# lim0606/pytorch-ardae-vae

Measured on AMD Instinct MI355X. Metric: AR-DAE-VAE train-steps/sec (batch 512, nz_cdae 256) on dbMNIST, higher is better.
Workload: dtype f32; 1 GPU; BASELINE config #2: MNISTIPVAE mlp z=32 h=256 + cDAE mlp-grad h=256 L=3, global batch 512, nz_cdae 256 (131072 rows), dynamic binarisation on device, 1 cDAE + 1 VAE update per step; global_batch=512, nz_cdae=256, per_gpu_batch=512, parallelism=dp1

## Files before the change

pytorch-ardae-vae_amd/csrc/linear_wide.hip:

```cpp
#include <string.h>

#include "linear_wide_kernel.h"

namespace ardae {
namespace wide {

int wide_grid(int ntiles, int ncp) {
  static const char* genv = debug_knob("ARDAE_WIDE_GRID");
  int g = genv ? atoi(genv) : 256;
  g -= g % ncp;
  return ntiles < g ? ntiles : g;
}

}

namespace {

using namespace wide;

bool al16w(const void* p) { return (reinterpret_cast<uintptr_t>(p) & 15) == 0; }

int wide_panels(const LinArgs& a, int& nch, int& nj) {
  if (a.nsrc != 1) return 0;
  if (a.src[0].K == 256) { nch = 8; nj = 2; return 4; }
  if (a.src[0].K == 32) { nch = 4; nj = 2; return 1; }
  if (a.src[0].K == 512) { nch = 8; nj = 1; return 8; }
  if (a.src[0].K == 1024) { nch = 8; nj = 1; return 16; }
  return 0;
}

template <int EPI, int ACT, bool F1, bool F2>
int launch_wide_nch(const LinArgs& a, hipStream_t st) {
  int nch = 0, nj = 0;
  const int np = wide_panels(a, nch, nj);
  if (np == 16) {
    if constexpr (ACT == ACT_SOFTPLUS && !F1 && (EPI == EPI_ACT || (EPI == EPI_DACT && !F2))) return launch_wide<8, 16, 1, EPI, ACT, F1, F2>(a, st);
    ARDAE_CHECK_ARG(false, "linear_wide: K = 1024 is instantiated for softplus ACT / DACT-without-Q epilogues only");
  }
  if (np == 8) return launch_wide<8, 8, 1, EPI, ACT, F1, F2>(a, st);
  if (nch == 4) return launch_wide<4, 1, 2, EPI, ACT, F1, F2>(a, st);
  return launch_wide<8, 4, 2, EPI, ACT, F1, F2>(a, st);
}

template <int EPI, int ACT>
int launch_wide_flags(const LinArgs& a, hipStream_t st) {
  if constexpr (EPI == EPI_ACT) {
    const bool y2 = a.Y2 != nullptr, rs = a.rowscale != nullptr;
    if (y2 && rs) return launch_wide_nch<EPI, ACT, true, true>(a, st);
    if (y2) return launch_wide_nch<EPI, ACT, true, false>(a, st);
    if (rs) return launch_wide_nch<EPI, ACT, false, true>(a, st);
    return launch_wide_nch<EPI, ACT, false, false>(a, st);
  } else if constexpr (EPI == EPI_DACT) {
    if (a.Q) return launch_wide_nch<EPI, ACT, true, false>(a, st);
    return launch_wide_nch<EPI, ACT, false, false>(a, st);
  } else {
    return launch_wide_nch<EPI, ACT, false, false>(a, st);
  }
}

}

bool linear_wide_eligible(const LinArgs& a, int epi) {
  int nch = 0, nj = 0;
  if (wide_panels(a, nch, nj) == 0) return false;
  const int wgcols = 128 * nj;
  if (a.M <= 0 || (a.M % WBM) || a.Nout <= 0 || (a.Nout % wgcols)) return false;
  if ((int64_t)(a.M / WBM) * (a.Nout / wgcols) < 128) return false;
  for (int s = 0; s < a.nsrc; ++s) {
    if (a.src[s].K % 32 || (a.src[s].ld & 3) || !al16w(a.src[s].x)) return false;
    if ((int64_t)a.src[s].ld * a.M * 4 >= (int64_t)1 << 32) return false;
  }
  if (epi == EPI_DAE_LOSS) return false;
  if (a.colsum && linear_row_tile(a.M, a.Nout) != WBM) return false;
  if (a.src[0].K == 1024) {
    if (a.act != ACT_SOFTPLUS) return false;
    if (!((epi == EPI_ACT && !a.Y2) || (epi == EPI_DACT && !a.Q))) return false;
  }
  if (a.act != ACT_NONE && a.act != ACT_RELU && a.act != ACT_SOFTPLUS) return false;
  if (epi == EPI_CHAIN && a.act != ACT_SOFTPLUS) return false;
  if (256 % (a.Nout / wgcols)) return false;
  if (epi == EPI_ACT && a.rowbias) {
    if (a.rows_per_group <= 0) return false;
    if (a.rows_per_group % WBM && (a.rows_per_group < WBM || a.M % a.rows_per_group || a.colsum)) return false;
  }
  if (epi == EPI_ACT && a.rowscale && !a.rowscale_w) return false;
  const int64_t ldmax = std::max<int64_t>({a.ldY, a.ldY2, a.ldS, a.ldR, a.ldQ});
  if (ldmax * a.M * 4 >= (int64_t)1 << 32) return false;
  return true;
}

bool linear_wide_layers_eligible(const LinArgs* L, int nl, int epi) {
  static const bool on = !(debug_knob("ARDAE_WIDE_LAYERS") && atoi(debug_knob("ARDAE_WIDE_LAYERS")) == 0);
  if (!on || nl < 2 || nl > WIDE_MAXL || !(epi == EPI_ACT || epi == EPI_DACT || epi == EPI_CHAIN)) return false;
  const LinArgs& f = L[0];
  if (f.act != ACT_SOFTPLUS && !(f.act == ACT_RELU && epi != EPI_CHAIN)) return false;
  for (int l = 0; l < nl; ++l) {
    const LinArgs& a = L[l];
    if (!linear_wide_eligible(a, epi)) return false;
    if (a.M != f.M || a.Nout != 256 || a.nsrc != 1 || a.src[0].K != 256 || a.act != f.act || !a.Y) return false;
    if (l > 0 && (a.src[0].x != L[l - 1].Y || a.src[0].ld != L[l - 1].ldY)) return false;
    if (epi == EPI_ACT && (a.rowbias || a.rowscale || a.Y2)) return false;
    if (epi == EPI_DACT && ((a.Q != nullptr) != (f.Q != nullptr))) return false;
    if (epi == EPI_CHAIN && (!a.Y2 || !a.R)) return false;
  }
  return true;
}

int launch_linear_wide_layers(const LinArgs* L, int nl, int epi, hipStream_t st) {
  ARDAE_CHECK_ARG(linear_wide_layers_eligible(L, nl, epi), "linear_wide_layers: run not eligible");
  const int act = L[0].act;
  if (epi == EPI_ACT) return act == ACT_SOFTPLUS ? launch_wide_layers<8, 4, 2, EPI_ACT, ACT_SOFTPLUS, false, false>(L, nl, st)
                                                 : launch_wide_layers<8, 4, 2, EPI_ACT, ACT_RELU, false, false>(L, nl, st);
  if (epi == EPI_CHAIN) return launch_wide_layers<8, 4, 2, EPI_CHAIN, ACT_SOFTPLUS, false, false>(L, nl, st);
  if (L[0].Q) return act == ACT_SOFTPLUS ? launch_wide_layers<8, 4, 2, EPI_DACT, ACT_SOFTPLUS, true, false>(L, nl, st)
                                         : launch_wide_layers<8, 4, 2, EPI_DACT, ACT_RELU, true, false>(L, nl, st);
  return act == ACT_SOFTPLUS ? launch_wide_layers<8, 4, 2, EPI_DACT, ACT_SOFTPLUS, false, false>(L, nl, st)
                             : launch_wide_layers<8, 4, 2, EPI_DACT, ACT_RELU, false, false>(L, nl, st);
}

int launch_linear_wide(const LinArgs& a, int epi, hipStream_t st) {
  switch (epi) {
    case EPI_ACT:
      if (a.act == ACT_NONE) return launch_wide_flags<EPI_ACT, ACT_NONE>(a, st);
      if (a.act == ACT_RELU) return launch_wide_flags<EPI_ACT, ACT_RELU>(a, st);
      if (a.act == ACT_SOFTPLUS) return launch_wide_flags<EPI_ACT, ACT_SOFTPLUS>(a, st);
      break;
    case EPI_DACT:
      if (a.act == ACT_NONE) return launch_wide_flags<EPI_DACT, ACT_NONE>(a, st);
      if (a.act == ACT_RELU) return launch_wide_flags<EPI_DACT, ACT_RELU>(a, st);
      if (a.act == ACT_SOFTPLUS) return launch_wide_flags<EPI_DACT, ACT_SOFTPLUS>(a, st);
      break;
    case EPI_CHAIN:
      if (a.act == ACT_SOFTPLUS) return launch_wide_flags<EPI_CHAIN, ACT_SOFTPLUS>(a, st);
      break;
  }
  ARDAE_CHECK_ARG(false, "linear_wide: unsupported epilogue/activation combination (epi=%d act=%d)", epi, a.act);
  return -1;
}

}
```

pytorch-ardae-vae_amd/csrc/linear_wide_kernel.h:

```cpp
#pragma once
#include <stdlib.h>

#include <algorithm>
#include <type_traits>

#include "linear.h"
#include "profile.h"

#define ARDAE_NT_LD " nt"
#define ARDAE_NT_ST " nt"
namespace ardae {
namespace wide {

constexpr int WBM = 64;
constexpr int WLDW = 68;
constexpr int WBUF_BYTES = WBM * WLDW * 4;
constexpr int NBUF = 3;

typedef __attribute__((address_space(3))) float lds_f32;

template <int OFF>
__device__ __forceinline__ void gload4(f32x4& dst, unsigned voff, const float* sbase) {
  asm volatile("s_nop 4\n\tglobal_load_dwordx4 %0, %1, %2 offset:%3" : "=v"(dst) : "v"(voff), "s"(sbase), "n"(OFF) : "memory");
}
template <int OFF, bool NOP = true>
__device__ __forceinline__ void gload1(float& dst, unsigned voff, const float* sbase) {
  if (NOP) asm volatile("s_nop 4\n\tglobal_load_dword %0, %1, %2 offset:%3" : "=v"(dst) : "v"(voff), "s"(sbase), "n"(OFF) : "memory");
  else asm volatile("global_load_dword %0, %1, %2 offset:%3" : "=v"(dst) : "v"(voff), "s"(sbase), "n"(OFF) : "memory");
}
template <bool NOP = true>
__device__ __forceinline__ void gstore1(unsigned voff, float v, float* sbase) {
  if (NOP) asm volatile("s_nop 4\n\tglobal_store_dword %0, %1, %2" ::"v"(voff), "v"(v), "s"(sbase) : "memory");
  else asm volatile("global_store_dword %0, %1, %2" ::"v"(voff), "v"(v), "s"(sbase) : "memory");
}
typedef int i32x4 __attribute__((ext_vector_type(4)));
__device__ __forceinline__ i32x4 make_rsrc(const void* p, unsigned bytes) {
  const unsigned long long a = (unsigned long long)p;
  i32x4 r;
  r[0] = (int)(unsigned)a;
  r[1] = (int)((unsigned)(a >> 32) & 0xffffu);
  r[2] = (int)bytes;
  r[3] = 0x00020000;
  return r;
}
template <int OFF, int H>
__device__ __forceinline__ void bload1(f32x2& dst, unsigned voff, const i32x4& rsrc, unsigned soff) {
  asm volatile("s_nop 4\n\tbuffer_load_dword %0, %1, %2, %3 offen offset:%4" ARDAE_NT_LD : "+v"(dst[H]) : "v"(voff), "s"(rsrc), "s"(soff), "n"(OFF) : "memory");
}
__device__ __forceinline__ void bstore1(unsigned voff, float v, const i32x4& rsrc, unsigned soff) {
  asm volatile("s_nop 4\n\tbuffer_store_dword %0, %1, %2, %3 offen" ARDAE_NT_ST ::"v"(v), "v"(voff), "s"(rsrc), "s"(soff) : "memory");
}
template <int OFF>
__device__ __forceinline__ void lds_read4(f32x4& dst, unsigned addr) {
  asm volatile("ds_read_b128 %0, %1 offset:%2" : "=v"(dst) : "v"(addr), "n"(OFF) : "memory");
}
template <int OFF>
__device__ __forceinline__ void lds_write4(unsigned addr, const f32x4& v) {
  asm volatile("ds_write_b128 %0, %1 offset:%2" ::"v"(addr), "v"(v), "n"(OFF) : "memory");
}
template <int VM, int NX>
__device__ __forceinline__ void wait_panel(f32x4 (&x)[NX]) {
  if (NX == 4) asm volatile("s_waitcnt vmcnt(%4)" : "+v"(x[0]), "+v"(x[1]), "+v"(x[2]), "+v"(x[3]) : "n"(VM) : "memory");
  else asm volatile("s_waitcnt vmcnt(%2)" : "+v"(x[0]), "+v"(x[1]) : "n"(VM) : "memory");
}
template <int VM>
__device__ __forceinline__ void wait16(f32x2* v) {
  asm volatile("s_waitcnt vmcnt(%8)" : "+v"(v[0]), "+v"(v[1]), "+v"(v[2]), "+v"(v[3]), "+v"(v[4]), "+v"(v[5]), "+v"(v[6]), "+v"(v[7]) : "n"(VM) : "memory");
}

template <int NCH>
struct PanelGeo {
  static constexpr int C4 = 2 * NCH;
  static constexpr int RPP = 256 / C4;
  static constexpr int NX = WBM / RPP;
};


template <int NCH, int NX>
__device__ __forceinline__ void store_panel(const f32x4 (&xv)[NX], unsigned waddr) {
  using PG = PanelGeo<NCH>;
  lds_write4<0>(waddr, xv[0]);
  lds_write4<PG::RPP * WLDW * 4>(waddr, xv[1]);
  if (NX == 4) {
    lds_write4<2 * PG::RPP * WLDW * 4>(waddr, xv[2]);
    lds_write4<3 * PG::RPP * WLDW * 4>(waddr, xv[3]);
  }
}
template <int OFF>
__device__ __forceinline__ void bload4(f32x4& dst, unsigned voff, const i32x4& rsrc, unsigned soff) {
  asm volatile("s_nop 4\n\tbuffer_load_dwordx4 %0, %1, %2, %3 offen offset:%4" : "=v"(dst) : "v"(voff), "s"(rsrc), "s"(soff), "n"(OFF) : "memory");
}
__device__ __forceinline__ void gload4_agpr(f32x4& dst, unsigned voff, const float* sbase) {
  asm volatile("s_nop 4\n\tglobal_load_dwordx4 %0, %1, %2" : "=a"(dst) : "v"(voff), "s"(sbase) : "memory");
}
template <int VM, int NJ>
__device__ __forceinline__ void wait_slab(f32x4 (&b)[NJ]) {
  if constexpr (NJ == 2) asm volatile("s_waitcnt vmcnt(%2)" : "+a"(b[0]), "+a"(b[1]) : "n"(VM) : "memory");
  else asm volatile("s_waitcnt vmcnt(%1)" : "+a"(b[0]) : "n"(VM) : "memory");
}
template <bool FIRST, bool LAST>
__device__ __forceinline__ void mfma_vab(f32x16& acc, float a, float b) {
  if (FIRST) asm volatile("v_mfma_f32_32x32x2_f32 %0, %1, %2, 0" : "=v"(acc) : "v"(a), "a"(b));
  else if (LAST) asm volatile("v_mfma_f32_32x32x2_f32 %0, %1, %2, %0\n\ts_nop 15\n\ts_nop 3" : "+v"(acc) : "v"(a), "a"(b));
  else asm volatile("v_mfma_f32_32x32x2_f32 %0, %1, %2, %0" : "+v"(acc) : "v"(a), "a"(b));
}

constexpr int wide_slots(int NCH, int NP, int NJ) { return (NJ * NCH * NP * 4 <= 256) ? NCH * NP : 64 / NJ; }

template <int NCH, int NP, int NJ, int NLT, int NST, bool HP>
struct Sched {
  static constexpr int NX = PanelGeo<NCH>::NX;
  static constexpr int G = NP * NCH;
  static constexpr int SLOTS = wide_slots(NCH, NP, NJ);
  static constexpr bool ROLL = SLOTS < G;
  static constexpr bool DEFER = NP >= 2;
  static constexpr int NSTO = (DEFER && HP) ? 32 * NJ * NST : 0;
  static constexpr int NLD = 32 * NJ * NLT;
  static constexpr int XW = NCH - 3, BAR = NCH - 2;
  static constexpr int GE = G >= 16 ? G - 5 : G - 1;
  static constexpr int GS = (NSTO + NLD) == 0 ? 0 : NLD == 0 ? GE : (GE * NSTO + (NSTO + NLD) / 2) / (NSTO + NLD);
  static constexpr int GRB = NLD == 0 ? GE - 1 : GS;
  static constexpr int DS = GS > 0 ? GS : 1, DL = GE > GS ? GE - GS : 1;
  static constexpr int st_lo(int g) { return g >= GS ? NSTO : NSTO * g / DS; }
  static constexpr int st_hi(int g) { return g >= GS ? NSTO : NSTO * (g + 1) / DS; }
  static constexpr int ld_lo(int g) { return g < GS ? 0 : g >= GE ? NLD : NLD * (g - GS) / DL; }
  static constexpr int ld_hi(int g) { return g < GS ? 0 : g >= GE ? NLD : NLD * (g - GS + 1) / DL; }
  static constexpr int n_rb(int g) { return g == GRB ? NJ : 0; }
  static constexpr int n_sl(int g) { return ROLL ? NJ : 0; }
  static constexpr int vmem(int g) { return (st_hi(g) - st_lo(g)) + n_rb(g) + (ld_hi(g) - ld_lo(g)) + n_sl(g); }
  static constexpr int vm_panel(int p) {
    int n = 0;
    for (int k = 0; k < XW; ++k) n += vmem(p * NCH + k);
    return n > 63 ? 63 : n;
  }
  static constexpr int vm_slab(int p, int c) {
    const int g = p * NCH + c;
    int n = ((ROLL ? SLOTS : G) - 1 - g) * NJ + NX * (c > 0 ? p + 1 : p);
    if (n < 0) n = 0;
    for (int k = 0; k < g; ++k) n += vmem(k);
    return n > 63 ? 63 : n;
  }
};

template <int EPI, int ACT, bool F1, bool F2, int NJ_ = 2>
struct WideEpi {
  static constexpr int NJ = NJ_;
  static constexpr int NLT = EPI == EPI_ACT ? (F2 ? 1 : 0) : EPI == EPI_DACT ? (F1 ? 2 : 1) : 2;
  static constexpr int NST = EPI == EPI_ACT ? (F1 ? 2 : 1) : EPI == EPI_DACT ? 1 : 2;
  static constexpr bool SIGMA_OPERAND = EPI == EPI_ACT;
  static constexpr bool CHAIN = EPI == EPI_CHAIN;

  const LinArgs& a;
  unsigned vY, vY2, vL0, vL1, vRS, vC;
  i32x4 rY, rY2, rL0, rL1, rRS;
  unsigned sY, sY2, sL0, sL1;
  float bcol0, wsig0, wfc0; unsigned pad_; float bcol1, wsig1, wfc1;
  int colw_loaded;

  __device__ __forceinline__ WideEpi(const LinArgs& a_, int lane) : a(a_), colw_loaded(-1) {
    const int l31 = lane & 31, hh = lane >> 5;
    vY = (unsigned)((4 * hh * a.ldY + l31) * 4);
    vY2 = NST == 2 ? (unsigned)((4 * hh * (a.Y2 ? a.ldY2 : a.ldY) + l31) * 4) : 0u;
    vL0 = (EPI != EPI_ACT) ? (unsigned)((4 * hh * a.ldS + l31) * 4) : 0u;
    vL1 = (EPI == EPI_CHAIN) ? (unsigned)((4 * hh * a.ldR + l31) * 4) : (EPI == EPI_DACT && F1) ? (unsigned)((4 * hh * a.ldQ + l31) * 4) : 0u;
    vRS = (unsigned)(16 * hh);
    vC = (unsigned)(l31 * 4);
    bcol0 = bcol1 = wsig0 = wsig1 = wfc0 = wfc1 = 0.f;
    const unsigned M = (unsigned)a.M;
    const float* y2 = a.Y2 ? a.Y2 : a.Y;
    const int ld2 = a.Y2 ? a.ldY2 : a.ldY;
    sY = (unsigned)a.ldY * 4u; sY2 = (unsigned)ld2 * 4u;
    rY = make_rsrc(a.Y, M * sY);
    rY2 = make_rsrc(y2, M * sY2);
    const float* t0 = EPI != EPI_ACT ? a.S : a.Y;
    const float* t1 = EPI == EPI_CHAIN ? a.R : (EPI == EPI_DACT && F1) ? a.Q : a.Y;
    sL0 = (unsigned)(EPI != EPI_ACT ? a.ldS : a.ldY) * 4u;
    sL1 = (unsigned)(EPI == EPI_CHAIN ? a.ldR : (EPI == EPI_DACT && F1) ? a.ldQ : a.ldY) * 4u;
    rL0 = make_rsrc(t0, M * sL0);
    rL1 = make_rsrc(t1, M * sL1);
    rRS = make_rsrc((EPI == EPI_ACT && a.rowscale) ? a.rowscale : a.src[0].x, M * 4u);
  }

  __device__ __forceinline__ void column_operands(int colw, int lane) {
    if (EPI != EPI_ACT || colw == colw_loaded) return;
    colw_loaded = colw;
    const int l31 = lane & 31;
#pragma unroll
    for (int j = 0; j < NJ; ++j) {
      const int col = colw + 32 * j + l31;
      const float b = a.bias ? a.bias[col] : 0.f;
      const float w = (F2 && a.rowscale_w) ? a.rowscale_w[col] : 0.f;
      const float f = (F1 && a.R) ? a.R[col] : 0.f;
      if (j == 0) { bcol0 = b; wsig0 = w; wfc0 = f; } else { bcol1 = b; wsig1 = w; wfc1 = f; }
    }
  }

  template <int JJ>
  __device__ __forceinline__ void issue_rowbias_one(float& rbj, int row0, int colw) const {
    const float* p = (EPI == EPI_ACT && a.rowbias) ? a.rowbias + (size_t)(row0 / a.rows_per_group) * a.rowbias_ld + colw
                                                     : a.Y + (size_t)row0 * a.ldY + colw;
    gload1<128 * JJ>(rbj, vC, p);
  }

  template <int HB>
  __device__ __forceinline__ void math(const f32x16& acc16, f32x2* l0, f32x2* l1, float brow, f32x2& csum) const {
    constexpr int J = HB >> 2, H = HB & 1;
    const float ws = J == 0 ? wsig0 : wsig1, nw = -(J == 0 ? wfc0 : wfc1);
    const f32x2 brow2 = {brow, brow}, wsig2 = {ws, ws}, nwfc2 = {nw, nw};
#pragma unroll
    for (int k = 0; k < 4; ++k) {
      f32x2 v;
      v[0] = acc16[8 * H + 2 * k];
      v[1] = acc16[8 * H + 2 * k + 1];
      f32x2 em;
      if (EPI == EPI_ACT) {
        f32x2 x = v + brow2;
        if (F2 && a.rowscale) x = l0[k] * wsig2 + x;
        const f32x2 y = act_fwd2<ACT>(x);
        if (NST == 2) l1[k] = (F1 && a.Y2) ? nwfc2 * act_d1_2<ACT>(y, em) : y;
        l0[k] = y;
      } else if (EPI == EPI_DACT) {
        const f32x2 d1 = act_d1_2<ACT>(l0[k], em);
        if (F1) asm volatile("v_pk_fma_f32 %0, %1, %2, %3" : "+v"(l0[k]) : "v"(v), "v"(d1), "v"(l1[k]));
        else asm volatile("v_pk_mul_f32 %0, %1, %2" : "+v"(l0[k]) : "v"(v), "v"(d1));
      } else {
        const f32x2 d1 = act_d1_2<ACT>(l0[k], em);
        const f32x2 vem = v * em;
        asm volatile("v_pk_mul_f32 %0, %1, %2" : "+v"(l0[k]) : "v"(v), "v"(d1));
        asm volatile("v_pk_mul_f32 %0, %1, %0" : "+v"(l1[k]) : "v"(vem));
      }
      csum += l0[k];
    }
  }

  template <int HB>
  __device__ __forceinline__ void stores(const f32x2* y, const f32x2* y2, int row0, int colw) const {
    constexpr int J = HB >> 2, I = (HB >> 1) & 1, H = HB & 1;
    const unsigned r0 = (unsigned)(row0 + 32 * I + 16 * H), c4 = (unsigned)(colw + 32 * J) * 4u;
    unsigned oy = r0 * sY + c4;
#pragma unroll
    for (int e = 0; e < 8; ++e) {
      bstore1(vY, y[e >> 1][e & 1], rY, oy);
      oy += (e == 3) ? 5u * sY : sY;
    }
    if (NST == 2) {
      unsigned o2 = r0 * sY2 + c4;
#pragma unroll
      for (int e = 0; e < 8; ++e) {
        bstore1(vY2, y2[e >> 1][e & 1], rY2, o2);
        o2 += (e == 3) ? 5u * sY2 : sY2;
      }
    }
  }

  __device__ __forceinline__ void store_all(const f32x2* y, const f32x2* y2, int row0, int colw) const {
    stores<0>(y + 0, y2 + 0, row0, colw); stores<1>(y + 4, y2 + 4, row0, colw); stores<2>(y + 8, y2 + 8, row0, colw);
    stores<3>(y + 12, y2 + 12, row0, colw);
    if constexpr (NJ == 2) {
      stores<4>(y + 16, y2 + 16, row0, colw); stores<5>(y + 20, y2 + 20, row0, colw);
      stores<6>(y + 24, y2 + 24, row0, colw); stores<7>(y + 28, y2 + 28, row0, colw);
    }
  }

  template <int VM, bool STORE_NOW>
  __device__ __forceinline__ void run(f32x16 (&acc)[2][NJ], f32x2* l0, f32x2* l1, float (&rb)[NJ], int lane, int row0, int colw, int tile_row) const {
    asm volatile("s_waitcnt vmcnt(%2)" : "+v"(rb[0]), "+v"(rb[NJ - 1]) : "n"(VM) : "memory");
    if (NLT >= 1) { wait16<VM>(l0); wait16<VM>(l0 + 8); if (NJ == 2) { wait16<VM>(l0 + 16); wait16<VM>(l0 + 24); } }
    if (NLT == 2) { wait16<VM>(l1); wait16<VM>(l1 + 8); if (NJ == 2) { wait16<VM>(l1 + 16); wait16<VM>(l1 + 24); } }
    const bool has_rb = EPI == EPI_ACT && a.rowbias != nullptr;
    const float br0 = bcol0 + (has_rb ? rb[0] : 0.f), br1 = bcol1 + (has_rb ? rb[NJ - 1] : 0.f);
    f32x2 csum[2] = {f32x2{0.f, 0.f}, f32x2{0.f, 0.f}};
    math<0>(acc[0][0], l0 + 0, l1 + 0, br0, csum[0]); __builtin_amdgcn_sched_barrier(0);
    math<1>(acc[0][0], l0 + 4, l1 + 4, br0, csum[0]); __builtin_amdgcn_sched_barrier(0);
    math<2>(acc[1][0], l0 + 8, l1 + 8, br0, csum[0]); __builtin_amdgcn_sched_barrier(0);
    math<3>(acc[1][0], l0 + 12, l1 + 12, br0, csum[0]); __builtin_amdgcn_sched_barrier(0);
    if constexpr (NJ == 2) {
      math<4>(acc[0][1], l0 + 16, l1 + 16, br1, csum[1]); __builtin_amdgcn_sched_barrier(0);
      math<5>(acc[0][1], l0 + 20, l1 + 20, br1, csum[1]); __builtin_amdgcn_sched_barrier(0);
      math<6>(acc[1][1], l0 + 24, l1 + 24, br1, csum[1]); __builtin_amdgcn_sched_barrier(0);
      math<7>(acc[1][1], l0 + 28, l1 + 28, br1, csum[1]); __builtin_amdgcn_sched_barrier(0);
    }
    if (STORE_NOW) store_all(l0, l1, row0, colw);
    if (a.colsum != nullptr) {
#pragma unroll
      for (int j = 0; j < NJ; ++j) {
        const float c1 = csum[j][0] + csum[j][1];
        const float c2 = c1 + __shfl_xor(c1, 32);
        if (lane < 32) a.colsum[(size_t)tile_row * a.Nout + colw + 32 * j + lane] = c2;
      }
    }
  }
};

template <int NCH, class EPI_T>
struct PanelCtx {
  const EPI_T& epi;
  const i32x4& rX;
  unsigned xvoff, xstep, xsoff_next;
  unsigned raddr, raddr_next, waddr_next;
  int row0, colw, prev_row0;
  const float* wslab;
  unsigned bvoff;
  int kch;
};

template <int C, int P, int NCH, int NP, bool HP, bool FT, class EPI_T>
struct ChunkOps {
  using SC = Sched<NCH, NP, EPI_T::NJ, EPI_T::NLT, EPI_T::NST, HP>;
  static constexpr int NX = PanelGeo<NCH>::NX;
  static constexpr int NLT = EPI_T::NLT, NST = EPI_T::NST, NJ = EPI_T::NJ, NMF = 8 * EPI_T::NJ;
  static constexpr int GC = P * NCH + C;
  static constexpr int n_a = 2, n_x = C == 0 ? NX : 0, n_w = C == SC::XW ? NX : 0, n_st = SC::st_hi(GC) - SC::st_lo(GC), n_rb = SC::n_rb(GC),
                       n_op = SC::ld_hi(GC) - SC::ld_lo(GC), n_sl = SC::n_sl(GC);
  static constexpr int o_a = 0, o_x = o_a + n_a, o_w = o_x + n_x, o_st = o_w + n_w, o_rb = o_st + n_st, o_op = o_rb + n_rb, o_sl = o_op + n_op,
                       total = o_sl + n_sl;
  static constexpr int SLOTS = SC::SLOTS;
  static constexpr int PER = (total + NMF - 1) / NMF;

  struct Ptrs {
    unsigned py, py2, p0, p1;
  };

  template <int K>
  static __device__ __forceinline__ void op(f32x4 (&A)[2][2], f32x4 (&Bw)[SC::SLOTS][EPI_T::NJ], f32x4 (&xv)[NX], f32x2* l0, f32x2* l1, float (&rb)[EPI_T::NJ],
                                            const PanelCtx<NCH, EPI_T>& x, Ptrs& q) {
    using PG = PanelGeo<NCH>;
    const EPI_T& ep = x.epi;
    if constexpr (K >= o_sl) {
      constexpr int j = K - o_sl, GP = (GC + SC::G - 1) % SC::G, GN = (GP + SLOTS) % SC::G;
      asm volatile("s_nop 4\n\tglobal_load_dwordx4 %0, %1, %2" : "+a"(Bw[GP % SLOTS][j]) : "v"(x.bvoff), "s"(x.wslab + ((size_t)j * x.kch + GN) * 256) : "memory");
    } else if constexpr (K < o_x) {
      constexpr int i = K - o_a;
      if constexpr (C + 1 < NCH) lds_read4<(C + 1) * 32 + i * 32 * WLDW * 4>(A[(C + 1) & 1][i], x.raddr);
      else lds_read4<i * 32 * WLDW * 4>(A[0][i], x.raddr_next);
    } else if constexpr (K < o_w) {
      constexpr int u = K - o_x;
      bload4<0>(xv[u], x.xvoff, x.rX, x.xsoff_next + (unsigned)u * x.xstep);
    } else if constexpr (K < o_st) {
      constexpr int u = K - o_w;
      if constexpr (u == 0) wait_panel<SC::vm_panel(P), NX>(xv);
      lds_write4<u * PG::RPP * WLDW * 4>(x.waddr_next, xv[u]);
    } else if constexpr (K < o_rb) {
      constexpr int idx = SC::st_lo(GC) + (K - o_st);
      constexpr int HB = idx / (8 * NST), tns = (idx / 8) % NST, e = idx % 8;
      constexpr int J = HB >> 2, I = (HB >> 1) & 1, H = HB & 1;
      constexpr bool fresh = e == 0 || K == o_st;
      constexpr int roff = 32 * I + 16 * H + (e & 3) + 8 * (e >> 2);
      if constexpr (tns == 0) {
        if constexpr (fresh) q.py = (unsigned)(x.prev_row0 + roff) * ep.sY + (unsigned)(x.colw + 32 * J) * 4u;
        bstore1(ep.vY, l0[4 * HB + (e >> 1)][e & 1], ep.rY, q.py);
        q.py += (e == 3) ? 5u * ep.sY : ep.sY;
      } else {
        if constexpr (fresh) q.py2 = (unsigned)(x.prev_row0 + roff) * ep.sY2 + (unsigned)(x.colw + 32 * J) * 4u;
        bstore1(ep.vY2, l1[4 * HB + (e >> 1)][e & 1], ep.rY2, q.py2);
        q.py2 += (e == 3) ? 5u * ep.sY2 : ep.sY2;
      }
    } else if constexpr (K < o_op) {
      constexpr int k = K - o_rb;
      if constexpr (k == 0) ep.template issue_rowbias_one<0>(rb[0], x.row0, x.colw);
      else ep.template issue_rowbias_one<1>(rb[NJ - 1], x.row0, x.colw);
    } else if constexpr (K < o_sl) {
      constexpr int idx = SC::ld_lo(GC) + (K - o_op);
      constexpr int HB = idx / (8 * NLT), tns = (idx / 8) % NLT, e = idx % 8;
      constexpr int J = HB >> 2, I = (HB >> 1) & 1, H = HB & 1;
      constexpr bool fresh = e == 0 || K == o_op;
      constexpr int roff = 32 * I + 16 * H + (e & 3) + 8 * (e >> 2);
      if constexpr (EPI_T::SIGMA_OPERAND) {
        constexpr int off = ((e & 3) + 8 * (e >> 2)) * 4;
        bload1<off, (e & 1)>(l0[4 * HB + (e >> 1)], ep.vRS, ep.rRS, (unsigned)(x.row0 + 32 * I + 16 * H) * 4u);
      } else if constexpr (tns == 0) {
        if constexpr (fresh) q.p0 = (unsigned)(x.row0 + roff) * ep.sL0 + (unsigned)(x.colw + 32 * J) * 4u;
        bload1<0, (e & 1)>(l0[4 * HB + (e >> 1)], ep.vL0, ep.rL0, q.p0);
        q.p0 += (e == 3) ? 5u * ep.sL0 : ep.sL0;
      } else {
        if constexpr (fresh) q.p1 = (unsigned)(x.row0 + roff) * ep.sL1 + (unsigned)(x.colw + 32 * J) * 4u;
        bload1<0, (e & 1)>(l1[4 * HB + (e >> 1)], ep.vL1, ep.rL1, q.p1);
        q.p1 += (e == 3) ? 5u * ep.sL1 : ep.sL1;
      }
    }
  }

  template <int S, int R = 0>
  static __device__ __forceinline__ void slot(f32x4 (&A)[2][2], f32x4 (&Bw)[SC::SLOTS][EPI_T::NJ], f32x4 (&xv)[NX], f32x2* l0, f32x2* l1, float (&rb)[EPI_T::NJ],
                                              const PanelCtx<NCH, EPI_T>& x, Ptrs& q) {
    if constexpr (R < PER && S * PER + R < total) {
      op<S * PER + R>(A, Bw, xv, l0, l1, rb, x, q);
      slot<S, R + 1>(A, Bw, xv, l0, l1, rb, x, q);
    }
  }

  template <int S>
  static __device__ __forceinline__ void steps(f32x16 (&acc)[2][EPI_T::NJ], f32x4 (&A)[2][2], f32x4 (&Bw)[wide_slots(NCH, NP, EPI_T::NJ)][EPI_T::NJ], f32x4 (&xv)[NX], f32x2* l0, f32x2* l1,
                                               float (&rb)[EPI_T::NJ], const PanelCtx<NCH, EPI_T>& x, Ptrs& q) {
    if constexpr (S < NMF) {
      constexpr int kq = S / (2 * NJ), i = (S / NJ) & 1, j = S % NJ;
      mfma_vab<GC == 0 && kq == 0, GC == NP * NCH - 1 && S == NMF - 1>(acc[i][j], A[C & 1][i][kq], Bw[GC % SLOTS][j][kq]);
      slot<S>(A, Bw, xv, l0, l1, rb, x, q);
      steps<S + 1>(acc, A, Bw, xv, l0, l1, rb, x, q);
    }
  }

  static __device__ __forceinline__ void run(f32x16 (&acc)[2][EPI_T::NJ], f32x4 (&A)[2][2], f32x4 (&Bw)[wide_slots(NCH, NP, EPI_T::NJ)][EPI_T::NJ], f32x4 (&xv)[NX], f32x2* l0, f32x2* l1,
                                             float (&rb)[EPI_T::NJ], const PanelCtx<NCH, EPI_T>& x) {
    asm volatile("s_waitcnt lgkmcnt(0)" : "+v"(A[C & 1][0]), "+v"(A[C & 1][1]) : : "memory");
    if constexpr (FT && GC < SLOTS) wait_slab<SC::vm_slab(P, C), NJ>(Bw[GC % SLOTS]);
    else if constexpr (SC::ROLL) wait_slab<63, NJ>(Bw[GC % SLOTS]);
    if (C == SC::BAR) __builtin_amdgcn_s_barrier();
    Ptrs q{0u, 0u, 0u, 0u};
    steps<0>(acc, A, Bw, xv, l0, l1, rb, x, q);
  }
};

template <int P, int NCH, int NP, bool HP, bool FT, class EPI_T>
__device__ __forceinline__ void panel(f32x16 (&acc)[2][EPI_T::NJ], f32x4 (&A)[2][2], f32x4 (&Bw)[wide_slots(NCH, NP, EPI_T::NJ)][EPI_T::NJ], f32x4 (&xv)[PanelGeo<NCH>::NX], f32x2* l0, f32x2* l1,
                                      float (&rb)[EPI_T::NJ], const PanelCtx<NCH, EPI_T>& x) {
  ChunkOps<0, P, NCH, NP, HP, FT, EPI_T>::run(acc, A, Bw, xv, l0, l1, rb, x);
  ChunkOps<1, P, NCH, NP, HP, FT, EPI_T>::run(acc, A, Bw, xv, l0, l1, rb, x);
  ChunkOps<2, P, NCH, NP, HP, FT, EPI_T>::run(acc, A, Bw, xv, l0, l1, rb, x);
  ChunkOps<3, P, NCH, NP, HP, FT, EPI_T>::run(acc, A, Bw, xv, l0, l1, rb, x);
  if constexpr (NCH == 8) {
    ChunkOps<4, P, NCH, NP, HP, FT, EPI_T>::run(acc, A, Bw, xv, l0, l1, rb, x);
    ChunkOps<5, P, NCH, NP, HP, FT, EPI_T>::run(acc, A, Bw, xv, l0, l1, rb, x);
    ChunkOps<6, P, NCH, NP, HP, FT, EPI_T>::run(acc, A, Bw, xv, l0, l1, rb, x);
    ChunkOps<7, P, NCH, NP, HP, FT, EPI_T>::run(acc, A, Bw, xv, l0, l1, rb, x);
  }
}

template <int P, int NCH, int NP, bool HP, bool FT, class EPI_T, class PX>
__device__ __forceinline__ void tile_panels(f32x16 (&acc)[2][EPI_T::NJ], f32x4 (&A)[2][2], f32x4 (&Bw)[wide_slots(NCH, NP, EPI_T::NJ)][EPI_T::NJ], f32x4 (&xv)[PanelGeo<NCH>::NX], f32x2* l0,
                                            f32x2* l1, float (&rb)[EPI_T::NJ], const EPI_T& epi, const i32x4& rX, unsigned xvoff, unsigned xstep, int& buf,
                                            unsigned rlane, unsigned wlane, int row0, int colw, int prev_row0, int tile, int tnext, const PX& panel_x,
                                            const float* wslab, unsigned bvoff, int kch) {
  if constexpr (P < NP) {
    constexpr bool lastp = P + 1 == NP;
    const int bnext = buf + 1 == NBUF ? 0 : buf + 1;
    const PanelCtx<NCH, EPI_T> x{epi, rX, xvoff, xstep, panel_x(lastp ? tnext : tile, lastp ? 0 : P + 1), rlane + buf * WBUF_BYTES, rlane + bnext * WBUF_BYTES,
                                 wlane + bnext * WBUF_BYTES, row0, colw, prev_row0, wslab, bvoff, kch};
    panel<P, NCH, NP, HP, FT>(acc, A, Bw, xv, l0, l1, rb, x);
    buf = bnext;
    tile_panels<P + 1, NCH, NP, HP, FT>(acc, A, Bw, xv, l0, l1, rb, epi, rX, xvoff, xstep, buf, rlane, wlane, row0, colw, prev_row0, tile, tnext, panel_x, wslab,
                                        bvoff, kch);
  }
}

template <int NCH, int NP, int NJ, int EPI, int ACT, bool F1, bool F2>
__device__ __forceinline__ void wide_body(const LinArgs& a, int nrt, int ncp, int tpg) {
  using PG = PanelGeo<NCH>;
  using EPI_T = WideEpi<EPI, ACT, F1, F2, NJ>;
  using SC = Sched<NCH, NP, NJ, EPI_T::NLT, EPI_T::NST, true>;
  constexpr int NX = PG::NX, G = NP * NCH;
  static_assert(NCH % 2 == 0 && NCH >= 4, "fragment double buffer / XW, BAR chunks");
  constexpr int SLOTS = wide_slots(NCH, NP, NJ);
  static_assert(NJ * SLOTS * 4 <= 256 && G % SLOTS == 0, "the slab window must fit the AGPR file");
  __shared__ float lds[NBUF * WBM * WLDW];

#ifdef ARDAE_STAMPS
  const unsigned long long r_kernel = __builtin_amdgcn_s_memrealtime();
#endif
  const int tid = threadIdx.x, lane = tid & 63;
  const int wave = __builtin_amdgcn_readfirstlane(tid >> 6);
  const int l31 = lane & 31, hh = lane >> 5;

  const unsigned lds0 = (unsigned)(uintptr_t)(lds_f32*)lds;
  const unsigned rlane = lds0 + (unsigned)((l31 * WLDW + hh * 4) * 4);
  const unsigned wlane = lds0 + (unsigned)(((tid / PG::C4) * WLDW + (tid % PG::C4) * 4) * 4);

  const int b = (int)blockIdx.x, nwg = (int)gridDim.x;
  const bool xcd_map = ncp > 1 && nwg % (8 * ncp) == 0;
  const int cp = xcd_map ? (b >> 3) % ncp : b % ncp;
  const int rt0 = xcd_map ? ((b >> 3) / ncp) * 8 + (b & 7) : b / ncp;
  const int rts = nwg / ncp;
  const int colw = (cp * 4 * NJ + wave * NJ) * 32;
  EPI_T epi(a, lane);
  epi.column_operands(colw, lane);

  const unsigned ldx4 = (unsigned)a.src[0].ld * 4u;
  const i32x4 rX = make_rsrc(a.src[0].x, (unsigned)a.M * ldx4);
  const unsigned xvoff = (unsigned)(tid / PG::C4) * ldx4 + (unsigned)(tid % PG::C4) * 16u;
  const unsigned xstep = (unsigned)PG::RPP * ldx4;
  auto tile_row0 = [&](int rt) -> int {
    if (tpg == 0) return rt * WBM;
    const int g = rt / tpg, j = rt - g * tpg;
    const int r = j * WBM, last = a.rows_per_group - WBM;
    return __builtin_amdgcn_readfirstlane(g * a.rows_per_group + (r < last ? r : last));
  };
  auto panel_x = [&](int rt, int p) -> unsigned { return (unsigned)tile_row0(rt) * ldx4 + (unsigned)(p * 8 * NCH) * 4u; };

  f32x4 A[2][2], Bw[SLOTS][NJ], xv[NX];
  f32x2 l0[16 * NJ], l1[16 * NJ];
  float rb[NJ];
#pragma unroll
  for (int i = 0; i < 16 * NJ; ++i) l0[i] = l1[i] = f32x2{0.f, 0.f};
  int tile = rt0;
  const unsigned bvoff = (unsigned)lane * 16u;
  const int kch = a.src[0].K >> 3;
  const float* wslab = a.src[0].wp + (size_t)(cp * 4 * NJ + wave * NJ) * kch * 256;
  {
    const float* wp = wslab;
    const unsigned x0 = panel_x(tile, 0);
#pragma unroll
    for (int u = 0; u < NX; ++u) bload4<0>(xv[u], xvoff, rX, x0 + (unsigned)u * xstep);
#pragma unroll
    for (int g = 0; g < SLOTS; ++g) {
      gload4_agpr(Bw[g][0], bvoff, wp + (size_t)g * 256);
      if constexpr (NJ == 2) gload4_agpr(Bw[g][1], bvoff, wp + ((size_t)kch + g) * 256);
    }
    wait_panel<(NJ * SLOTS > 63 ? 63 : NJ * SLOTS), NX>(xv);
    store_panel<NCH, NX>(xv, wlane);
    asm volatile("s_waitcnt lgkmcnt(0)" ::: "memory");
    __builtin_amdgcn_s_barrier();
    lds_read4<0>(A[0][0], rlane);
    lds_read4<32 * WLDW * 4>(A[0][1], rlane);
  }
  int buf = 0;
  int prev_row0 = -1;
#ifdef ARDAE_STAMPS
  unsigned long long t_k = 0, t_e = 0;
  const unsigned long long t_begin = __builtin_amdgcn_s_memtime();
  const unsigned long long r_begin = __builtin_amdgcn_s_memrealtime();
#endif
  auto do_tile = [&](auto ft_tag) {
    constexpr bool FT = decltype(ft_tag)::value, HP = SC::DEFER && !FT;
#ifdef ARDAE_STAMPS
    const unsigned long long T0 = __builtin_amdgcn_s_memtime();
#endif
    const int tr = tile;
    const int row0 = tile_row0(tr);
    const int tnext = tile + rts < nrt ? tile + rts : tile;
    f32x16 acc[2][NJ];
    tile_panels<0, NCH, NP, HP, FT>(acc, A, Bw, xv, l0, l1, rb, epi, rX, xvoff, xstep, buf, rlane, wlane, row0, colw, prev_row0, tile, tnext, panel_x, wslab, bvoff,
                                    kch);
#ifdef ARDAE_STAMPS
    const unsigned long long T1 = __builtin_amdgcn_s_memtime();
    t_k += T1 - T0;
#endif
    asm volatile("s_waitcnt vmcnt(0) lgkmcnt(0)"
                 : "+v"(A[0][0]), "+v"(A[0][1]), "+v"(acc[0][0]), "+v"(acc[0][NJ - 1]), "+v"(acc[1][0]), "+v"(acc[1][NJ - 1])
                 :
                 : "memory");
    epi.template run<0, !SC::DEFER>(acc, l0, l1, rb, lane, row0, colw, tr);
    if (SC::DEFER) prev_row0 = row0;
#ifdef ARDAE_STAMPS
    t_e += __builtin_amdgcn_s_memtime() - T1;
#endif
  };
  do_tile(std::true_type{});
  for (tile += rts; tile < nrt; tile += rts) do_tile(std::false_type{});
  if (SC::DEFER && prev_row0 >= 0) epi.store_all(l0, l1, prev_row0, colw);
  asm volatile("s_waitcnt vmcnt(0) lgkmcnt(0)" ::: "memory");
#ifdef ARDAE_STAMPS
  if (a.tile_loss != nullptr && lane == 0) {
    unsigned long long* o = reinterpret_cast<unsigned long long*>(a.tile_loss) + ((size_t)blockIdx.x * 4 + wave) * 8;
    const unsigned long long r_end = __builtin_amdgcn_s_memrealtime();
    o[0] = t_k; o[1] = t_e; o[2] = __builtin_amdgcn_s_memtime() - t_begin; o[3] = r_end - r_begin;
    o[4] = r_begin; o[5] = r_end; o[6] = r_kernel;
  }
#endif
}

template <int NCH, int NP, int NJ, int EPI, int ACT, bool F1, bool F2>
__global__ __launch_bounds__(256, 1) void linear_wide_kernel(const LinArgs a, int nrt, int ncp, int tpg) {
  wide_body<NCH, NP, NJ, EPI, ACT, F1, F2>(a, nrt, ncp, tpg);
}

constexpr int WIDE_MAXL = 6;
struct WideLayers {
  int nl;
  LinArgs L[WIDE_MAXL];
};
template <int NCH, int NP, int NJ, int EPI, int ACT, bool F1, bool F2>
__global__ __launch_bounds__(256, 1) void linear_wide_layers_kernel(const WideLayers c, int nrt, int ncp, int tpg) {
  for (int l = 0; l < c.nl; ++l) {
    wide_body<NCH, NP, NJ, EPI, ACT, F1, F2>(c.L[l], nrt, ncp, tpg);
    __syncthreads();
  }
}

int wide_grid(int ntiles, int ncp);

template <int NCH, int NP, int NJ, int EPI, int ACT, bool F1, bool F2>
int launch_wide(const LinArgs& a, hipStream_t st) {
  const int ncp = a.Nout / (128 * NJ);
  const int tpg = (EPI == EPI_ACT && a.rowbias && a.rows_per_group % WBM) ? (a.rows_per_group + WBM - 1) / WBM : 0;
  const int nrt = tpg ? (a.M / a.rows_per_group) * tpg : a.M / WBM;
  const int ntiles = nrt * ncp;
  const int grid = wide_grid(ntiles, ncp);
  if (g_prof_enabled) {
    char name[96];
    snprintf(name, sizeof(name), "linear_wide_kernel<%d, %d, %d, %d, %d, %s, %s>", NCH, NP, NJ, EPI, ACT, F1 ? "true" : "false", F2 ? "true" : "false");
    double ksum = 0;
    for (int s = 0; s < a.nsrc; ++s) ksum += a.src[s].K;
    double tensors = 1.0 + (a.Y2 ? 1 : 0) + ((EPI == EPI_DACT || EPI == EPI_CHAIN) ? 1 : 0) + ((EPI == EPI_CHAIN) ? 1 : 0) +
                     ((EPI == EPI_DACT && a.Q) ? 1 : 0);
    prof_begin(st, name, 2.0 * a.M * (double)a.Nout * ksum, 4.0 * ((double)a.M * ksum + tensors * a.M * (double)a.Nout + ksum * a.Nout));
  }
  hipLaunchKernelGGL((linear_wide_kernel<NCH, NP, NJ, EPI, ACT, F1, F2>), dim3(grid), dim3(256), 0, st, a, nrt, ncp, tpg);
  prof_end(st);
  ARDAE_LAUNCH_CHECK();
  return 0;
}


template <int NCH, int NP, int NJ, int EPI, int ACT, bool F1, bool F2>
int launch_wide_layers(const LinArgs* L, int nl, hipStream_t st) {
  const LinArgs& a = L[0];
  const int ncp = a.Nout / (128 * NJ);
  const int nrt = a.M / WBM;
  const int grid = wide_grid(nrt * ncp, ncp);
  WideLayers c;
  memset(&c, 0, sizeof(c));
  c.nl = nl;
  for (int l = 0; l < nl; ++l) c.L[l] = L[l];
  if (g_prof_enabled) {
    char name[112];
    snprintf(name, sizeof(name), "linear_wide_layers_kernel<%d, %d, %d, %d, %d, %s, %s> x%d", NCH, NP, NJ, EPI, ACT, F1 ? "true" : "false", F2 ? "true" : "false", nl);
    double fl = 0, by = 0;
    for (int l = 0; l < nl; ++l) {
      const double K = L[l].src[0].K;
      const double tensors = 1.0 + (L[l].Y2 ? 1 : 0) + ((EPI == EPI_DACT || EPI == EPI_CHAIN) ? 1 : 0) + ((EPI == EPI_CHAIN) ? 1 : 0) + ((EPI == EPI_DACT && L[l].Q) ? 1 : 0);
      fl += 2.0 * a.M * (double)a.Nout * K;
      by += 4.0 * ((double)a.M * K + tensors * a.M * (double)a.Nout + K * a.Nout);
    }
    prof_begin(st, name, fl, by);
  }
  hipLaunchKernelGGL((linear_wide_layers_kernel<NCH, NP, NJ, EPI, ACT, F1, F2>), dim3(grid), dim3(256), 0, st, c, nrt, ncp, 0);
  prof_end(st);
  ARDAE_LAUNCH_CHECK();
  return 0;
}

#define ARDAE_WIDE_LAYERS_FOR(X)                          \
  X(8, 4, 2, EPI_ACT, ACT_SOFTPLUS, false, false)         \
  X(8, 4, 2, EPI_ACT, ACT_RELU, false, false)             \
  X(8, 4, 2, EPI_DACT, ACT_SOFTPLUS, false, false)        \
  X(8, 4, 2, EPI_DACT, ACT_SOFTPLUS, true, false)         \
  X(8, 4, 2, EPI_DACT, ACT_RELU, false, false)            \
  X(8, 4, 2, EPI_DACT, ACT_RELU, true, false)             \
  X(8, 4, 2, EPI_CHAIN, ACT_SOFTPLUS, false, false)
#define ARDAE_WIDE_LAYERS_EXTERN(NCH, NP, NJ, EPI, ACT, F1, F2) extern template int launch_wide_layers<NCH, NP, NJ, EPI, ACT, F1, F2>(const LinArgs*, int, hipStream_t);
#define ARDAE_WIDE_LAYERS_INSTANTIATE(NCH, NP, NJ, EPI, ACT, F1, F2) template int launch_wide_layers<NCH, NP, NJ, EPI, ACT, F1, F2>(const LinArgs*, int, hipStream_t);
#ifndef ARDAE_WIDE_INST_TU
ARDAE_WIDE_LAYERS_FOR(ARDAE_WIDE_LAYERS_EXTERN)
#endif

#define ARDAE_WIDE_FOR_GEOS(X, EPI, ACT, F1, F2) \
  X(8, 4, 2, EPI, ACT, F1, F2)                    \
  X(4, 1, 2, EPI, ACT, F1, F2)                    \
  X(8, 8, 1, EPI, ACT, F1, F2)
#define ARDAE_WIDE_FOR_ACT_FLAGS(X, ACT)          \
  ARDAE_WIDE_FOR_GEOS(X, EPI_ACT, ACT, false, false) \
  ARDAE_WIDE_FOR_GEOS(X, EPI_ACT, ACT, false, true)  \
  ARDAE_WIDE_FOR_GEOS(X, EPI_ACT, ACT, true, false)  \
  ARDAE_WIDE_FOR_GEOS(X, EPI_ACT, ACT, true, true)
#define ARDAE_WIDE_FOR_DACT_FLAGS(X, ACT)          \
  ARDAE_WIDE_FOR_GEOS(X, EPI_DACT, ACT, false, false) \
  ARDAE_WIDE_FOR_GEOS(X, EPI_DACT, ACT, true, false)
#define ARDAE_WIDE_FOR_K1024(X)                        \
  X(8, 16, 1, EPI_ACT, ACT_SOFTPLUS, false, false)     \
  X(8, 16, 1, EPI_ACT, ACT_SOFTPLUS, false, true)      \
  X(8, 16, 1, EPI_DACT, ACT_SOFTPLUS, false, false)
#define ARDAE_WIDE_EXTERN(NCH, NP, NJ, EPI, ACT, F1, F2) extern template int launch_wide<NCH, NP, NJ, EPI, ACT, F1, F2>(const LinArgs&, hipStream_t);
#define ARDAE_WIDE_INSTANTIATE(NCH, NP, NJ, EPI, ACT, F1, F2) template int launch_wide<NCH, NP, NJ, EPI, ACT, F1, F2>(const LinArgs&, hipStream_t);
#ifndef ARDAE_WIDE_INST_TU
ARDAE_WIDE_FOR_ACT_FLAGS(ARDAE_WIDE_EXTERN, ACT_NONE)
ARDAE_WIDE_FOR_ACT_FLAGS(ARDAE_WIDE_EXTERN, ACT_RELU)
ARDAE_WIDE_FOR_ACT_FLAGS(ARDAE_WIDE_EXTERN, ACT_SOFTPLUS)
ARDAE_WIDE_FOR_DACT_FLAGS(ARDAE_WIDE_EXTERN, ACT_NONE)
ARDAE_WIDE_FOR_DACT_FLAGS(ARDAE_WIDE_EXTERN, ACT_RELU)
ARDAE_WIDE_FOR_DACT_FLAGS(ARDAE_WIDE_EXTERN, ACT_SOFTPLUS)
ARDAE_WIDE_FOR_GEOS(ARDAE_WIDE_EXTERN, EPI_CHAIN, ACT_SOFTPLUS, false, false)
ARDAE_WIDE_FOR_K1024(ARDAE_WIDE_EXTERN)
#endif

}
}
```

Measured before the change: 219.5 train-steps/sec.

## Fuse heterogeneous layer runs into one persistent wide-layers kernel

Adds a mixed-variant layers kernel that switches the wide GEMM body per layer at runtime: rowbias/rowscale/Y2 epilogue flags for forward passes, and a K=32 first layer for tangent chain passes. Softplus runs that were previously split into several launches can now run as a single persistent launch with block-level syncs between layers. LDS allocation moves to the kernel entry so the different body instantiations share one buffer. The cost is more code in one kernel, possibly higher register pressure, and a runtime branch per layer.

```diff
diff --git a/pytorch-ardae-vae_amd/csrc/linear_wide.hip b/pytorch-ardae-vae_amd/csrc/linear_wide.hip
--- a/pytorch-ardae-vae_amd/csrc/linear_wide.hip
+++ b/pytorch-ardae-vae_amd/csrc/linear_wide.hip
@@ -89,26 +89,55 @@
   return true;
 }
 
+namespace {
+
+int wide_layers_mode() {
+  static const int mode = [] {
+    const char* e = debug_knob("ARDAE_WIDE_LAYERS");
+    if (!e) return 2;
+    const int v = atoi(e);
+    return v == 0 ? 0 : v == 1 ? 1 : 2;
+  }();
+  return mode;
+}
+
+bool wide_layers_homogeneous(const LinArgs* L, int nl, int epi) {
+  for (int l = 0; l < nl; ++l) {
+    const LinArgs& a = L[l];
+    if (a.src[0].K != 256) return false;
+    if (epi == EPI_ACT && (a.rowbias || a.rowscale || a.Y2)) return false;
+  }
+  return true;
+}
+
+}
+
 bool linear_wide_layers_eligible(const LinArgs* L, int nl, int epi) {
-  static const bool on = !(debug_knob("ARDAE_WIDE_LAYERS") && atoi(debug_knob("ARDAE_WIDE_LAYERS")) == 0);
-  if (!on || nl < 2 || nl > WIDE_MAXL || !(epi == EPI_ACT || epi == EPI_DACT || epi == EPI_CHAIN)) return false;
+  const int mode = wide_layers_mode();
+  if (mode == 0 || nl < 2 || nl > WIDE_MAXL || !(epi == EPI_ACT || epi == EPI_DACT || epi == EPI_CHAIN)) return false;
   const LinArgs& f = L[0];
   if (f.act != ACT_SOFTPLUS && !(f.act == ACT_RELU && epi != EPI_CHAIN)) return false;
   for (int l = 0; l < nl; ++l) {
     const LinArgs& a = L[l];
     if (!linear_wide_eligible(a, epi)) return false;
-    if (a.M != f.M || a.Nout != 256 || a.nsrc != 1 || a.src[0].K != 256 || a.act != f.act || !a.Y) return false;
+    if (a.M != f.M || a.Nout != 256 || a.nsrc != 1 || a.act != f.act || !a.Y) return false;
+    if (a.src[0].K != 256 && !(epi == EPI_CHAIN && l == 0 && a.src[0].K == 32)) return false;
     if (l > 0 && (a.src[0].x != L[l - 1].Y || a.src[0].ld != L[l - 1].ldY)) return false;
-    if (epi == EPI_ACT && (a.rowbias || a.rowscale || a.Y2)) return false;
+    if (epi == EPI_ACT && a.rowbias && (a.rows_per_group <= 0 || a.rows_per_group % WBM)) return false;
     if (epi == EPI_DACT && ((a.Q != nullptr) != (f.Q != nullptr))) return false;
     if (epi == EPI_CHAIN && (!a.Y2 || !a.R)) return false;
+    for (int k = 0; k < nl; ++k)
+      if (a.rowbias && (a.rowbias == L[k].Y || a.rowbias == L[k].Y2)) return false;
   }
+  if (!wide_layers_homogeneous(L, nl, epi) && (mode < 2 || f.act != ACT_SOFTPLUS)) return false;
   return true;
 }
 
 int launch_linear_wide_layers(const LinArgs* L, int nl, int epi, hipStream_t st) {
   ARDAE_CHECK_ARG(linear_wide_layers_eligible(L, nl, epi), "linear_wide_layers: run not eligible");
   const int act = L[0].act;
+  if (!wide_layers_homogeneous(L, nl, epi))
+    return epi == EPI_ACT ? launch_wide_layers_mixed<EPI_ACT, ACT_SOFTPLUS>(L, nl, st) : launch_wide_layers_mixed<EPI_CHAIN, ACT_SOFTPLUS>(L, nl, st);
   if (epi == EPI_ACT) return act == ACT_SOFTPLUS ? launch_wide_layers<8, 4, 2, EPI_ACT, ACT_SOFTPLUS, false, false>(L, nl, st)
                                                  : launch_wide_layers<8, 4, 2, EPI_ACT, ACT_RELU, false, false>(L, nl, st);
   if (epi == EPI_CHAIN) return launch_wide_layers<8, 4, 2, EPI_CHAIN, ACT_SOFTPLUS, false, false>(L, nl, st);
diff --git a/pytorch-ardae-vae_amd/csrc/linear_wide_inst_layers_mix_act.hip b/pytorch-ardae-vae_amd/csrc/linear_wide_inst_layers_mix_act.hip
--- /dev/null
+++ b/pytorch-ardae-vae_amd/csrc/linear_wide_inst_layers_mix_act.hip
@@ -0,0 +1,10 @@
+#define ARDAE_WIDE_INST_TU
+#include <string.h>
+
+#include "linear_wide_kernel.h"
+
+namespace ardae {
+namespace wide {
+template int launch_wide_layers_mixed<EPI_ACT, ACT_SOFTPLUS>(const LinArgs*, int, hipStream_t);
+}
+}
diff --git a/pytorch-ardae-vae_amd/csrc/linear_wide_inst_layers_mix_chain.hip b/pytorch-ardae-vae_amd/csrc/linear_wide_inst_layers_mix_chain.hip
--- /dev/null
+++ b/pytorch-ardae-vae_amd/csrc/linear_wide_inst_layers_mix_chain.hip
@@ -0,0 +1,10 @@
+#define ARDAE_WIDE_INST_TU
+#include <string.h>
+
+#include "linear_wide_kernel.h"
+
+namespace ardae {
+namespace wide {
+template int launch_wide_layers_mixed<EPI_CHAIN, ACT_SOFTPLUS>(const LinArgs*, int, hipStream_t);
+}
+}
diff --git a/pytorch-ardae-vae_amd/csrc/linear_wide_kernel.h b/pytorch-ardae-vae_amd/csrc/linear_wide_kernel.h
--- a/pytorch-ardae-vae_amd/csrc/linear_wide_kernel.h
+++ b/pytorch-ardae-vae_amd/csrc/linear_wide_kernel.h
@@ -16,6 +16,7 @@
 constexpr int WLDW = 68;
 constexpr int WBUF_BYTES = WBM * WLDW * 4;
 constexpr int NBUF = 3;
+constexpr int WIDE_LDS_FLOATS = NBUF * WBM * WLDW;
 
 typedef __attribute__((address_space(3))) float lds_f32;
 
@@ -444,7 +445,7 @@
 }
 
 template <int NCH, int NP, int NJ, int EPI, int ACT, bool F1, bool F2>
-__device__ __forceinline__ void wide_body(const LinArgs& a, int nrt, int ncp, int tpg) {
+__device__ __forceinline__ void wide_body(const LinArgs& a, unsigned lds0, int tid, int nrt, int ncp, int tpg) {
   using PG = PanelGeo<NCH>;
   using EPI_T = WideEpi<EPI, ACT, F1, F2, NJ>;
   using SC = Sched<NCH, NP, NJ, EPI_T::NLT, EPI_T::NST, true>;
@@ -452,16 +453,14 @@
   static_assert(NCH % 2 == 0 && NCH >= 4, "fragment double buffer / XW, BAR chunks");
   constexpr int SLOTS = wide_slots(NCH, NP, NJ);
   static_assert(NJ * SLOTS * 4 <= 256 && G % SLOTS == 0, "the slab window must fit the AGPR file");
-  __shared__ float lds[NBUF * WBM * WLDW];
 
 #ifdef ARDAE_STAMPS
   const unsigned long long r_kernel = __builtin_amdgcn_s_memrealtime();
 #endif
-  const int tid = threadIdx.x, lane = tid & 63;
+  const int lane = tid & 63;
   const int wave = __builtin_amdgcn_readfirstlane(tid >> 6);
   const int l31 = lane & 31, hh = lane >> 5;
 
-  const unsigned lds0 = (unsigned)(uintptr_t)(lds_f32*)lds;
   const unsigned rlane = lds0 + (unsigned)((l31 * WLDW + hh * 4) * 4);
   const unsigned wlane = lds0 + (unsigned)(((tid / PG::C4) * WLDW + (tid % PG::C4) * 4) * 4);
 
@@ -560,18 +559,52 @@
 
 template <int NCH, int NP, int NJ, int EPI, int ACT, bool F1, bool F2>
 __global__ __launch_bounds__(256, 1) void linear_wide_kernel(const LinArgs a, int nrt, int ncp, int tpg) {
-  wide_body<NCH, NP, NJ, EPI, ACT, F1, F2>(a, nrt, ncp, tpg);
+  __shared__ float lds[WIDE_LDS_FLOATS];
+  wide_body<NCH, NP, NJ, EPI, ACT, F1, F2>(a, (unsigned)(uintptr_t)(lds_f32*)lds, (int)threadIdx.x, nrt, ncp, tpg);
 }
 
 constexpr int WIDE_MAXL = 6;
 struct WideLayers {
   int nl;
+  int var[WIDE_MAXL];
   LinArgs L[WIDE_MAXL];
 };
 template <int NCH, int NP, int NJ, int EPI, int ACT, bool F1, bool F2>
 __global__ __launch_bounds__(256, 1) void linear_wide_layers_kernel(const WideLayers c, int nrt, int ncp, int tpg) {
+  __shared__ float lds[WIDE_LDS_FLOATS];
+  const unsigned lds0 = (unsigned)(uintptr_t)(lds_f32*)lds;
   for (int l = 0; l < c.nl; ++l) {
-    wide_body<NCH, NP, NJ, EPI, ACT, F1, F2>(c.L[l], nrt, ncp, tpg);
+    wide_body<NCH, NP, NJ, EPI, ACT, F1, F2>(c.L[l], lds0, (int)threadIdx.x, nrt, ncp, tpg);
+    __syncthreads();
+  }
+}
+
+inline int wide_variant(const LinArgs& a, int epi) {
+  if (epi == EPI_ACT) return (a.Y2 ? 2 : 0) + (a.rowscale ? 1 : 0);
+  return a.src[0].K == 32 ? 1 : 0;
+}
+template <int EPI, int ACT>
+__global__ __launch_bounds__(256, 1) void linear_wide_layers_kernel(const WideLayers c, int nrt) {
+  static_assert(EPI == EPI_ACT || EPI == EPI_CHAIN, "mixed runs: forward and tangent passes");
+  __shared__ float lds[WIDE_LDS_FLOATS];
+  const unsigned lds0 = (unsigned)(uintptr_t)(lds_f32*)lds;
+  const int wave = __builtin_amdgcn_readfirstlane((int)threadIdx.x >> 6);
+  for (int l = 0; l < c.nl; ++l) {
+    const int v = c.var[l];
+    int lane;
+    asm volatile("v_mbcnt_lo_u32_b32 %0, -1, 0\n\tv_mbcnt_hi_u32_b32 %0, -1, %0" : "=v"(lane));
+    const int tid = wave * 64 + lane;
+    if constexpr (EPI == EPI_ACT) {
+      switch (v) {
+        case 0: wide_body<8, 4, 2, EPI, ACT, false, false>(c.L[l], lds0, tid, nrt, 1, 0); break;
+        case 1: wide_body<8, 4, 2, EPI, ACT, false, true>(c.L[l], lds0, tid, nrt, 1, 0); break;
+        case 2: wide_body<8, 4, 2, EPI, ACT, true, false>(c.L[l], lds0, tid, nrt, 1, 0); break;
+        default: wide_body<8, 4, 2, EPI, ACT, true, true>(c.L[l], lds0, tid, nrt, 1, 0); break;
+      }
+    } else {
+      if (v == 1) wide_body<4, 1, 2, EPI, ACT, false, false>(c.L[l], lds0, tid, nrt, 1, 0);
+      else wide_body<8, 4, 2, EPI, ACT, false, false>(c.L[l], lds0, tid, nrt, 1, 0);
+    }
     __syncthreads();
   }
 }
@@ -600,6 +633,16 @@
   return 0;
 }
 
+inline void wide_layers_work(const LinArgs* L, int nl, int epi, double& fl, double& by) {
+  fl = by = 0;
+  for (int l = 0; l < nl; ++l) {
+    const LinArgs& a = L[l];
+    const double K = a.src[0].K;
+    const double tensors = 1.0 + (a.Y2 ? 1 : 0) + ((epi == EPI_DACT || epi == EPI_CHAIN) ? 1 : 0) + ((epi == EPI_CHAIN) ? 1 : 0) + ((epi == EPI_DACT && a.Q) ? 1 : 0);
+    fl += 2.0 * a.M * (double)a.Nout * K;
+    by += 4.0 * ((double)a.M * K + tensors * a.M * (double)a.Nout + K * a.Nout);
+  }
+}
 
 template <int NCH, int NP, int NJ, int EPI, int ACT, bool F1, bool F2>
 int launch_wide_layers(const LinArgs* L, int nl, hipStream_t st) {
@@ -614,13 +657,8 @@
   if (g_prof_enabled) {
     char name[112];
     snprintf(name, sizeof(name), "linear_wide_layers_kernel<%d, %d, %d, %d, %d, %s, %s> x%d", NCH, NP, NJ, EPI, ACT, F1 ? "true" : "false", F2 ? "true" : "false", nl);
-    double fl = 0, by = 0;
-    for (int l = 0; l < nl; ++l) {
-      const double K = L[l].src[0].K;
-      const double tensors = 1.0 + (L[l].Y2 ? 1 : 0) + ((EPI == EPI_DACT || EPI == EPI_CHAIN) ? 1 : 0) + ((EPI == EPI_CHAIN) ? 1 : 0) + ((EPI == EPI_DACT && L[l].Q) ? 1 : 0);
-      fl += 2.0 * a.M * (double)a.Nout * K;
-      by += 4.0 * ((double)a.M * K + tensors * a.M * (double)a.Nout + K * a.Nout);
-    }
+    double fl, by;
+    wide_layers_work(L, nl, EPI, fl, by);
     prof_begin(st, name, fl, by);
   }
   hipLaunchKernelGGL((linear_wide_layers_kernel<NCH, NP, NJ, EPI, ACT, F1, F2>), dim3(grid), dim3(256), 0, st, c, nrt, ncp, 0);
@@ -628,6 +666,37 @@
   ARDAE_LAUNCH_CHECK();
   return 0;
 }
+
+template <int EPI, int ACT>
+int launch_wide_layers_mixed(const LinArgs* L, int nl, hipStream_t st) {
+  const int nrt = L[0].M / WBM;
+  WideLayers c;
+  memset(&c, 0, sizeof(c));
+  c.nl = nl;
+  for (int l = 0; l < nl; ++l) {
+    ARDAE_CHECK_ARG(L[l].Nout == 256 && L[l].M == L[0].M && L[l].M % WBM == 0, "linear_wide_layers: layer %d of a mixed run has another tile map", l);
+    ARDAE_CHECK_ARG(!(EPI == EPI_ACT && L[l].rowbias && L[l].rows_per_group % WBM), "linear_wide_layers: layer %d needs group tiles", l);
+    ARDAE_CHECK_ARG(L[l].src[0].K == 256 || (EPI == EPI_CHAIN && l == 0 && L[l].src[0].K == 32), "linear_wide_layers: layer %d: K = %d", l, L[l].src[0].K);
+    c.L[l] = L[l];
+    c.var[l] = wide_variant(L[l], EPI);
+  }
+  const int grid = wide_grid(nrt, 1);
+  if (g_prof_enabled) {
+    char name[112];
+    snprintf(name, sizeof(name), "linear_wide_layers_kernel<%d, %d> x%d", EPI, ACT, nl);
+    double fl, by;
+    wide_layers_work(L, nl, EPI, fl, by);
+    prof_begin(st, name, fl, by);
+  }
+  hipLaunchKernelGGL((linear_wide_layers_kernel<EPI, ACT>), dim3(grid), dim3(256), 0, st, c, nrt);
+  prof_end(st);
+  ARDAE_LAUNCH_CHECK();
+  return 0;
+}
+#ifndef ARDAE_WIDE_INST_TU
+extern template int launch_wide_layers_mixed<EPI_ACT, ACT_SOFTPLUS>(const LinArgs*, int, hipStream_t);
+extern template int launch_wide_layers_mixed<EPI_CHAIN, ACT_SOFTPLUS>(const LinArgs*, int, hipStream_t);
+#endif
 
 #define ARDAE_WIDE_LAYERS_FOR(X)                          \
   X(8, 4, 2, EPI_ACT, ACT_SOFTPLUS, false, false)         \
```

New measurement: 220.9 train-steps/sec, median of 6. About the same (+0.7%).
